# dfdazac/blp

Measured on AMD Instinct MI355X. Metric: scored triples/sec, all-entity eval (raw + filtered ranks, MRR + Hits@k), higher is better.
Workload: dtype f32; 1 GPU; fb15k237-transe; rel_model=transe, entities=14541, dim=128, triples_per_ranking_call=52870, filter_graph_edges=310116, parallelism=single GPU, ranks_in_process_group=1

## Files before the change

### blp_amd/csrc/rank_sad.hip

```cpp
#include <hip/hip_runtime.h>
#include <stddef.h>
#include <stdint.h>
#include <stdlib.h>

#include "exact_coop.h"
#include "knobs.h"
#include "launch.h"
#include "rank_common.h"
#include "sad_common.h"
#include "score_core.h"

#pragma clang fp contract(off)

namespace blp {


template <int D>
__global__ __launch_bounds__(256) void sad_range_kernel(const float* __restrict__ table, int64_t N, int64_t ld,
                                                        const QRows q_fixed,
                                                        const QRows q_rel, int64_t q_head, int64_t Q,
                                                        SadParams* __restrict__ partial) {
    SadRange range;
    const int64_t stride = (int64_t)gridDim.x * blockDim.x, t0 = (int64_t)blockIdx.x * blockDim.x + threadIdx.x;
    for (int64_t i = t0; i < N * (D / 4); i += stride) {
        const float4 v = *reinterpret_cast<const float4*>(table + (i / (D / 4)) * ld + (i % (D / 4)) * 4);
        range.see(v.x); range.see(v.y); range.see(v.z); range.see(v.w);
    }
    for (int64_t u = t0; u < Q * (D / 4); u += stride) {
        const bool head = u / (D / 4) < q_head;
        const float4 f = *reinterpret_cast<const float4*>(q_fixed.flat(4 * u, D));
        const float4 r = *reinterpret_cast<const float4*>(q_rel.flat(4 * u, D));
        range.see(sad_coef(f.x, r.x, head)); range.see(sad_coef(f.y, r.y, head));
        range.see(sad_coef(f.z, r.z, head)); range.see(sad_coef(f.w, r.w, head));
    }
    sad_range_block_store(range, partial);
}

constexpr int64_t kSFoldFinishBlocks = 1024;
constexpr int64_t kSFoldRangeBlocks = 256;

template <int D>
__device__ __forceinline__ void sad_quantize_table_tile(int64_t tile, const float* __restrict__ table, int64_t N,
                                                        int64_t ld, const SadParams* __restrict__ p,
                                                        uint4* __restrict__ cimg, unsigned* __restrict__ resid) {
    const SadScale sc = sad_scale(p);
    if (!sc.ok) return;
    const int row_in = threadIdx.x >> 2, part = threadIdx.x & 3;
    const int64_t row = tile * 64 + row_in;
    constexpr int F = D / 4;
    unsigned w[F / 2];
    float res = 0.f;
    bool outside = false;
    if (row < N) {
        const float* src = table + row * ld + part * F;
#pragma unroll
        for (int i = 0; i < F / 4; ++i) {
            const float4 v = *reinterpret_cast<const float4*>(src + 4 * i);
            w[2 * i] = sad_quant(v.x, sc, res, outside);
            w[2 * i] |= sad_quant(v.y, sc, res, outside) << 16;
            w[2 * i + 1] = sad_quant(v.z, sc, res, outside);
            w[2 * i + 1] |= sad_quant(v.w, sc, res, outside) << 16;
        }
    } else {
#pragma unroll
        for (int i = 0; i < F / 2; ++i) w[i] = 0;
    }
    res += __shfl_xor(res, 1);
    res += __shfl_xor(res, 2);
    outside |= (bool)__shfl_xor((int)outside, 1);
    outside |= (bool)__shfl_xor((int)outside, 2);
    if (part == 0)
        resid[row] = outside ? kSRowExact : (unsigned)(res * 1.0001f + kSResidSlack * D) + 1u;
    uint4* dst = cimg + (tile * (D / 8) + part * (F / 8)) * 64 + row_in;
#pragma unroll
    for (int i = 0; i < F / 8; ++i) dst[i * 64] = make_uint4(w[4 * i], w[4 * i + 1], w[4 * i + 2], w[4 * i + 3]);
}

template <int D>
__device__ __forceinline__ void sad_quantize_queries_block(int64_t vblock, int64_t vgrid, const QRows& q_fixed,
                                                           const QRows& q_rel, int64_t q_head,
                                                           int64_t Q, const float* __restrict__ key_true,
                                                           const SadParams* __restrict__ p,
                                                           unsigned* __restrict__ qimg,
                                                           int2* __restrict__ thr, unsigned* __restrict__ flags,
                                                           int64_t n_flag_words) {
    const int64_t i = vblock * 256 + threadIdx.x;
    for (int64_t j = i; j < n_flag_words; j += vgrid * 256) flags[j] = 0;
    const SadScale sc = sad_scale(p);
    if (!sc.ok) return;
    __shared__ float part_res[4], part_max[4];
    __shared__ int part_out[4];
    const bool live = i < Q * (D / 2);
    const int64_t q = live ? i / (D / 2) : Q - 1;
    const bool head = q < q_head;
    float res = 0.f, qmax = 0.f;
    bool outside = false;
    if (live) {
        const float2 f = *reinterpret_cast<const float2*>(q_fixed.flat(2 * i, D));
        const float2 r = *reinterpret_cast<const float2*>(q_rel.flat(2 * i, D));
        unsigned w = sad_quant(sad_coef(f.x, r.x, head), sc, res, outside);
        w |= sad_quant(sad_coef(f.y, r.y, head), sc, res, outside) << 16;
        qimg[i] = w;
        qmax = fmaxf(fmaxf(fabsf(f.x), fabsf(f.y)), fmaxf(fabsf(r.x), fabsf(r.y)));
    }
#pragma unroll
    for (int off = 1; off < (D / 2 < 64 ? D / 2 : 64); off <<= 1) {
        res += __shfl_xor(res, off);
        qmax = fmaxf(qmax, __shfl_xor(qmax, off));
        outside |= (bool)__shfl_xor((int)outside, off);
    }
    if constexpr (D / 2 > 64) {
        const int w = threadIdx.x >> 6;
        if ((threadIdx.x & 63) == 0) { part_res[w] = res; part_max[w] = qmax; part_out[w] = outside; }
        __syncthreads();
        res = part_res[w & ~1] + part_res[w | 1];
        qmax = fmaxf(part_max[w & ~1], part_max[w | 1]);
        outside = part_out[w & ~1] || part_out[w | 1];
    }
    if (live && i % (D / 2) == 0) {
        const double u = 5.9604644775390625e-8;
        const double dt = -(double)key_true[q], s = (double)sc.scale;
        const double M = (double)fmaxf(sad_range_maxabs(sc), qmax);
        const double band = (double)res * 1.0001 + 2.0 * kSResidSlack * D + 1.0;
        const double gamma = 1.05 * (D + 2) * u, rho = 6.0 * D * u * M;
        int t_lo = -1, t_hi = (int)kSThrMax;
        if (!outside && M < 3.0e38 && dt >= 0.0 && dt < 1.0e300) {
            const double lo_v = s * (dt - rho) / (1.0 + gamma) - band;
            const double hi_v = s * (dt + rho) / (1.0 - gamma) + band;
            if (lo_v > 2.0) t_lo = lo_v - 1.0 < (double)kSThrMax ? (int)(lo_v - 1.0) : (int)kSThrMax;
            if (hi_v + 2.0 < (double)kSThrMax) t_hi = (int)(hi_v + 2.0);
        }
        thr[q] = make_int2(t_lo, t_hi);
    }
}

template <int D>
__global__ __launch_bounds__(256) void sad_quantize_kernel(const float* __restrict__ table, int64_t N, int64_t ld,
                                                           SadParams* __restrict__ p, const SadParams* __restrict__ partial,
                                                           int n_partial, uint4* __restrict__ cimg,
                                                           unsigned* __restrict__ resid, unsigned table_blocks,
                                                           const QRows q_fixed, const QRows q_rel, int64_t q_head, int64_t Q,
                                                           const float* __restrict__ key_true, unsigned* __restrict__ qimg,
                                                           int2* __restrict__ thr, unsigned* __restrict__ flags,
                                                           int64_t n_flag_words) {
    __shared__ SadParams p_block;
    const SadParams* pp = p;
    if (n_partial > 0) {
        if (threadIdx.x < 64) {
            const SadParams r = sad_range_finish_wave(partial, n_partial, threadIdx.x);
            if (threadIdx.x == 0) {
                p_block = r;
                if (blockIdx.x == 0) *p = r;
            }
        }
        __syncthreads();
        pp = &p_block;
    }
    if (blockIdx.x < table_blocks)
        sad_quantize_table_tile<D>(blockIdx.x, table, N, ld, pp, cimg, resid);
    else
        sad_quantize_queries_block<D>(blockIdx.x - table_blocks, gridDim.x - table_blocks, q_fixed, q_rel, q_head, Q, key_true, pp,
                                      qimg, thr, flags, n_flag_words);
}

template <int D, int TPW>
struct SadTiles {
    unsigned v[TPW][D / 2];
    unsigned bias[TPW];
    unsigned long long exact_rows[TPW];
};

#ifndef BLP_SAD_CHUNK_BLOCK
#define BLP_SAD_CHUNK_BLOCK 4
#endif
constexpr unsigned kSadChunkBlock = BLP_SAD_CHUNK_BLOCK;

#ifndef BLP_SAD_INLINE_CAP
#define BLP_SAD_INLINE_CAP 256
#endif
constexpr unsigned kSInlineCap = BLP_SAD_INLINE_CAP;
static_assert(kSInlineCap <= kSQuota, "the pooled list is the four slices of pair_s");

#ifdef BLP_TIMING
__device__ unsigned long long g_sad_timing[4];
extern "C" int blp_debug_read_sad_timing(unsigned long long* out) {
    hipError_t err = hipMemcpyFromSymbol(out, HIP_SYMBOL(g_sad_timing), sizeof(g_sad_timing));
    unsigned long long zero[4] = {0, 0, 0, 0};
    if (err == hipSuccess) err = hipMemcpyToSymbol(HIP_SYMBOL(g_sad_timing), zero, sizeof(zero));
    return (int)err;
}
#endif

template <int D, int TPW>
__global__ __launch_bounds__(kSW * 64, (TPW * D / 2 <= 64 ? 5 : TPW * D / 2 <= 128 ? 3 : 2)) void rank_sad_kernel(
    const uint4* __restrict__ cimg, const unsigned* __restrict__ resid, int64_t n_rows, int n_groups, int q_per_group,
    const unsigned* __restrict__ qimg, const int2* __restrict__ thr, int64_t Q, int words_per_query,
    unsigned long long* __restrict__ acc,
    unsigned* __restrict__ flags, uint2* __restrict__ pairs, SadParams* __restrict__ params,
    const float* __restrict__ table, int64_t ld, const QRows q_fixed, const QRows q_rel, int64_t q_head,
    const float* __restrict__ key_true) {
    if (!sad_scale(params).ok) return;
#ifdef BLP_TIMING
    const unsigned long long clk0 = __builtin_readcyclecounter(), wall0 = __builtin_amdgcn_s_memrealtime();
#endif
    __shared__ int2 thr_s[kSChunk];
    __shared__ unsigned cnt[kSChunk];
    __shared__ uint2 pair_s[kSQuota];
    __shared__ unsigned wave_used[kSW], wave_base[kSW], ec_max_s;
    const int tid = threadIdx.x;
    const int wave = __builtin_amdgcn_readfirstlane(tid >> 6);
    const int lane = tid & 63;
    const unsigned n_blocks = gridDim.x, xcd = blockIdx.x & 7u, per_xcd = n_blocks >> 3, rem_b = n_blocks & 7u;
    const unsigned logical = (xcd < rem_b ? xcd * (per_xcd + 1) : rem_b * (per_xcd + 1) + (xcd - rem_b) * per_xcd) + (blockIdx.x >> 3);
    const unsigned n_chunks_all = n_blocks / (unsigned)n_groups;
    const unsigned per_cb = (unsigned)n_groups * kSadChunkBlock, cb = logical / per_cb, in_cb = logical % per_cb;
    const unsigned chunks_here = n_chunks_all - cb * kSadChunkBlock < kSadChunkBlock ? n_chunks_all - cb * kSadChunkBlock : kSadChunkBlock;
    const int group = (int)(in_cb / chunks_here);
    const int64_t q0 = (int64_t)(cb * kSadChunkBlock + in_cb % chunks_here) * q_per_group;
    const int nq = (int)(Q - q0 < q_per_group ? Q - q0 : q_per_group);

    for (int i = tid; i < kSChunk; i += kSW * 64) cnt[i] = 0;
    if (tid == 0) ec_max_s = 0;
    __syncthreads();

    SadTiles<D, TPW> c;
    const int64_t n_tiles = (n_rows + 63) / 64;
    const int64_t tile0 = ((int64_t)group * kSW + wave) * TPW;
    unsigned ec_max = 0;
    static_for<TPW>([&](auto tt) {
        constexpr int t = decltype(tt)::value;
        int64_t tile = tile0 + t;
        const bool exists = tile * 64 + lane < n_rows;
        tile = tile < n_tiles ? tile : n_tiles - 1;
        const unsigned ec = resid[tile * 64 + lane];
        const bool marked = exists && ec == kSRowExact;
        c.exact_rows[t] = __ballot(marked);
        c.bias[t] = exists ? (marked ? 0u : ec) : kSInvalid;
        ec_max = exists && !marked && ec > ec_max ? ec : ec_max;
        const uint4* src = cimg + tile * (D / 8) * 64 + lane;
        static_for<D / 8>([&](auto jj) {
            constexpr int j = decltype(jj)::value;
            const uint4 x = src[j * 64];
            c.v[t][4 * j] = x.x; c.v[t][4 * j + 1] = x.y; c.v[t][4 * j + 2] = x.z; c.v[t][4 * j + 3] = x.w;
        });
    });
#pragma unroll
    for (int off = 32; off > 0; off >>= 1) {
        const unsigned o = __shfl_xor(ec_max, off);
        ec_max = o > ec_max ? o : ec_max;
    }
    if (lane == 0) atomicMax(&ec_max_s, ec_max);
    __syncthreads();
    for (int i = tid; i < kSChunk; i += kSW * 64) {
        int2 t2 = i < nq ? thr[q0 + i] : make_int2(0, 0);
        const long long hi2 = (long long)t2.y + 2ll * ec_max_s;
        t2.y = hi2 < (long long)kSThrMax ? (int)hi2 : (int)kSThrMax;
        thr_s[i] = t2;
    }
    __syncthreads();

    unsigned my_pairs = 0;
    const float* row = reinterpret_cast<const float*>(qimg + q0 * (D / 2));
    sf16 cur = sload16<0>(row);
    sdrain(cur);
    for (int jb = 0; jb < nq; jb += 64) {
    const int jn = nq - jb < 64 ? nq - jb : 64;
    unsigned cnt_reg = 0;
    unsigned long long bit = 1;
    for (int j = jb; j < jb + jn; ++j, row += D / 2, bit <<= 1) {
        const float* next_row = row + D / 2;
        const int2 th = thr_s[j];
        unsigned sad[TPW];
        static_for<TPW>([&](auto tt) { sad[decltype(tt)::value] = c.bias[decltype(tt)::value]; });
        static_for<D / 32>([&](auto kk) {
            constexpr int k = decltype(kk)::value;
            sf16 nxt;
            if constexpr (k + 1 < D / 32) nxt = sload16<(k + 1) * 64>(row); else nxt = sload16<0>(next_row);
            if constexpr (k == 0) { if ((j & 3) == wave) stouch<D * 2>(row + 3 * (D / 2)); }
            static_for<16>([&](auto ii) {
                constexpr int i = decltype(ii)::value;
                const float qf = cur[i];
                const unsigned qv = __float_as_uint(qf);
                static_for<TPW>([&](auto tt) {
                    constexpr int t = decltype(tt)::value;
                    sad[t] = __builtin_amdgcn_sad_u16(qv, c.v[t][16 * k + i], sad[t]);
                });
            });
            sdrain(nxt);
            cur = nxt;
        });
        unsigned n_above = 0;
        static_for<TPW>([&](auto tt) {
            constexpr int t = decltype(tt)::value;
            const unsigned long long above = __ballot((int)sad[t] < th.x) & ~c.exact_rows[t];
            const unsigned long long und = (__ballot((int)sad[t] <= th.y) | c.exact_rows[t]) & ~above;
            unsigned n_t = __popcll(above);
            if (und) {
                const unsigned n = __popcll(und);
                if (my_pairs + n <= kSQuota / kSW) {
                    if ((und >> lane) & 1ull)
                        pair_s[wave * (kSQuota / kSW) + my_pairs + __popcll(und & ((1ull << lane) - 1ull))] =
                            make_uint2((unsigned)(q0 + j), (unsigned)((tile0 + t) * 64 + lane));
                    my_pairs += n;
                } else {
                    const int64_t tile = tile0 + t;
                    if (lane == 0) atomicOr(flags + (size_t)(q0 + j) * words_per_query + (tile >> 5), 1u << (tile & 31));
                    n_t = 0;
                }
            }
            n_above += n_t;
        });
        {
            unsigned long long saved;
            asm volatile("s_mov_b64 %1, exec\n\ts_mov_b64 exec, %3\n\tv_add_u32 %0, %0, %2\n\ts_mov_b64 exec, %1"
                         : "+v"(cnt_reg), "=&s"(saved) : "s"(n_above), "s"(bit));
        }
    }
    if (cnt_reg) atomicAdd(&cnt[jb + lane], cnt_reg);
    }
    __syncthreads();
    for (int i = tid; i < nq; i += kSW * 64) {
        const unsigned long long v = cnt[i];
        if (v) atomicAdd(acc + q0 + i, v | (v << 32));
    }
    if (lane == 0) wave_used[wave] = my_pairs;
    __syncthreads();
    unsigned start[kSW + 1];
    start[0] = 0;
#pragma unroll
    for (int w = 0; w < kSW; ++w) start[w + 1] = start[w] + __builtin_amdgcn_readfirstlane(wave_used[w]);
    const unsigned total = start[kSW];
    if (tid == 0 && total) atomicAdd(&params->n_listed, total);
    if (total <= kSInlineCap) {
        if (wave == 0) {
            for (unsigned base = 0; base < total; base += 64) {
                const bool live = base + lane < total;
                const unsigned t = live ? base + lane : base;
                const unsigned w = (unsigned)(t >= start[1]) + (unsigned)(t >= start[2]) + (unsigned)(t >= start[3]);
                const unsigned first = w == 0 ? start[0] : w == 1 ? start[1] : w == 2 ? start[2] : start[3];
                const uint2 p = pair_s[w * (kSQuota / kSW) + (t - first)];
                const int64_t q = p.x;
                const float key = transe_key_lane<D>(table + (int64_t)p.y * ld, q_fixed.row(q), q_rel.row(q), q < q_head);
                const float kt = key_true[q];
                const unsigned long long gt = live && key > kt, ge_ = live && key >= kt;
                if (gt | ge_) atomicAdd(acc + q, gt | (ge_ << 32));
            }
        }
    } else {
        if (tid == 0) {
            const unsigned base = atomicAdd(&params->n_pairs, total);
            for (int w = 0; w < kSW; ++w) wave_base[w] = base + start[w];
        }
        __syncthreads();
        for (int w = 0; w < kSW; ++w)
            for (unsigned i = tid; i < wave_used[w]; i += kSW * 64) pairs[wave_base[w] + i] = pair_s[w * (kSQuota / kSW) + i];
    }
#ifdef BLP_TIMING
    if (lane == 0) {
        atomicAdd(&g_sad_timing[0], __builtin_readcyclecounter() - clk0);
        atomicAdd(&g_sad_timing[1], __builtin_amdgcn_s_memrealtime() - wall0);
        atomicAdd(&g_sad_timing[2], 1ull);
    }
#endif
}

template <int D>
__global__ __launch_bounds__(64) void sad_refine_pairs_kernel(const float* __restrict__ table, int64_t ld,
                                                              const QRows q_fixed,
                                                              const QRows q_rel,
                                                              const float* __restrict__ key_true, int64_t q_head,
                                                              const uint2* __restrict__ pairs,
                                                              const SadParams* __restrict__ params,
                                                              unsigned long long* __restrict__ acc, const Gate gate) {
    if (gate_heavy(gate)) return;
    __shared__ __attribute__((aligned(16))) float slab[64 * kRefStride];
    const int lane = threadIdx.x;
    const int64_t n = params->n_pairs;
    for (int64_t base = (int64_t)blockIdx.x * 64; base < n; base += (int64_t)gridDim.x * 64) {
        const int64_t i = base + lane;
        const uint2 p = i < n ? pairs[i] : make_uint2(kSNoPair, 0u);
        const bool live = p.x != kSNoPair;
        const int64_t q = live ? p.x : 0;
        const bool head = q < q_head;
        const float key = transe_key_64<D>(table + (live ? (int64_t)p.y : 0) * ld, q_fixed.row(q), q_rel.row(q), head, slab, lane);
        const float kt = key_true[q];
        const unsigned long long gt = live && key > kt, ge_ = live && key >= kt;
        if (gt | ge_) atomicAdd(acc + q, gt | (ge_ << 32));
    }
}

template <int D>
__global__ __launch_bounds__(256) void sad_refine_tiles_kernel(const float* __restrict__ table, int64_t n_rows,
                                                               int64_t ld, const QRows q_fixed,
                                                               const QRows q_rel,
                                                               const float* __restrict__ key_true, int64_t q_head,
                                                               int64_t Q, int words_per_query,
                                                               const unsigned* __restrict__ flags,
                                                               const SadParams* __restrict__ params,
                                                               unsigned long long* __restrict__ acc, const Gate gate,
                                                               const FallbackPrep prep, int64_t q_tail) {
    if (gate_heavy(gate)) {
        fallback_prep<TRANSE, D>(prep, q_fixed, q_rel, q_head, q_tail);
        return;
    }
    __shared__ int list[kSweepQueries], n_list;
    const bool all = !sad_scale(params).ok;
    const int lane = threadIdx.x & 63;
    const int64_t q_base = (int64_t)blockIdx.x * kSweepQueries;
    const int n = flagged_queries(flags, q_base, Q, words_per_query, all, list, &n_list);
    for (int i = threadIdx.x >> 6; i < n; i += 4) {
    const int64_t q = q_base + list[i];
    const unsigned* row = flags + q * words_per_query;
    const float kt = key_true[q];
    const float* f = q_fixed.row(q);
    const float* rl = q_rel.row(q);
    unsigned gt = 0, ge = 0;
    for (int w0 = 0; w0 < words_per_query; w0 += 64) {
        const unsigned mine = w0 + lane < words_per_query ? (all ? 0xFFFFFFFFu : row[w0 + lane]) : 0u;
        unsigned long long nonzero = __ballot(mine != 0);
        while (nonzero) {
            const int src = __builtin_ctzll(nonzero);
            nonzero &= nonzero - 1;
            unsigned bits = __shfl(mine, src);
            const int64_t tile_base = (int64_t)(w0 + src) * 32;
            while (bits) {
                const int b = __builtin_ctz(bits);
                bits &= bits - 1;
                const int64_t r = (tile_base + b) * 64 + lane;
                const bool ok = r < n_rows;
                if (__ballot(ok) == 0) continue;
                float e[D];
                load_row<D>(e, table + (ok ? r : 0) * ld);
                const float key = q < q_head ? Scorer<TRANSE, HEAD, D>::template score<false>(e, LazyCoef<TRANSE, HEAD, D>{f, rl})
                                             : Scorer<TRANSE, TAIL, D>::template score<false>(e, LazyCoef<TRANSE, TAIL, D>{f, rl});
                gt += ok && key > kt;
                ge += ok && key >= kt;
            }
        }
    }
    if (__ballot(gt | ge) == 0) continue;
#pragma unroll
    for (int off = 32; off > 0; off >>= 1) {
        gt += __shfl_down(gt, off);
        ge += __shfl_down(ge, off);
    }
    if (lane == 0) atomicAdd(acc + q, (unsigned long long)gt | ((unsigned long long)ge << 32));
    }
}

static constexpr int sad_tiles_per_wave(int D) { return D <= 64 ? 2 : 1; }

struct SadWorkspace {
    float* key_true;
    unsigned long long* acc;
    SadParams* params; SadParams* partial; int2* thr; unsigned* qimg; uint4* cimg; unsigned* resid; unsigned* flags;
    uint2* pairs;
    float* fallback_coef;
    int64_t pass_groups;
    size_t bytes;
};

static int sad_queries_per_group(int D, int64_t N, int64_t Q) {
    const int64_t tiles_per_group = kSW * sad_tiles_per_wave(D);
    const int64_t n_groups = ((N + 63) / 64 + tiles_per_group - 1) / tiles_per_group;
    const int64_t resident = D >= 256 ? 256 * 3 : 256 * 5;
    const int64_t query_cycles = (int64_t)(D / 2) * sad_tiles_per_wave(D) * 17 / 4, setup_cycles = 12000;
    if (const int forced = (int)knob(KNOB_SAD_QUERIES_PER_GROUP))
        if (forced >= 16 && forced <= kSChunk && (forced & (forced - 1)) == 0) return forced;
    int best = kSChunk;
    int64_t best_cost = INT64_MAX;
    for (int per_group = kSChunk; per_group >= 16; per_group >>= 1) {
        const int64_t grid = n_groups * ((Q + per_group - 1) / per_group);
        const int64_t cost = ((grid + resident - 1) / resident) * (setup_cycles + per_group * query_cycles);
        if (cost < best_cost) { best_cost = cost; best = per_group; }
    }
    return best;
}

static int64_t sad_groups_per_pass(int D, int64_t N, int64_t Q) {
    const int64_t tiles_per_group = kSW * sad_tiles_per_wave(D);
    const int64_t n_groups = ((N + 63) / 64 + tiles_per_group - 1) / tiles_per_group;
    const int64_t per_group = sad_queries_per_group(D, N, Q);
    const int64_t n_chunks = (Q + per_group - 1) / per_group;
    const int64_t cap = (int64_t)256 << 20;
    int64_t by_pairs = cap / (kSQuota * 8) / (n_chunks > 0 ? n_chunks : 1);
    int64_t by_flags = cap / 4 / (Q > 0 ? Q : 1) * 32 / tiles_per_group;
    int64_t g = n_groups;
    if (g > by_pairs) g = by_pairs;
    if (g > by_flags) g = by_flags;
    if (const int64_t forced = knob(KNOB_SAD_PASS_GROUPS))
        if (forced > 0 && forced < g) g = forced;
    return g < 1 ? 1 : g;
}

static SadWorkspace carve_sad(void* base, int D, int64_t N, int64_t q_head, int64_t q_tail) {
    SadWorkspace w;
    const int64_t Q = q_head + q_tail;
    char* p = static_cast<char*>(base);
    size_t off = 0;
    w.key_true = reinterpret_cast<float*>(p + off);  off = align_up(off + (size_t)Q * 4, 256);
    w.acc = reinterpret_cast<unsigned long long*>(p + off);   off = align_up(off + (size_t)Q * 8, 256);
    w.params = reinterpret_cast<SadParams*>(p + off); off = align_up(off + sizeof(SadParams), 256);
    w.partial = reinterpret_cast<SadParams*>(p + off); off = align_up(off + sizeof(SadParams) * kSRangeBlocks, 256);
    w.thr = reinterpret_cast<int2*>(p + off);         off = align_up(off + (size_t)Q * 8, 256);
    w.qimg = reinterpret_cast<unsigned*>(p + off);    off = align_up(off + (size_t)(Q + 4) * (D / 2) * 4 + 64, 256);
    w.cimg = reinterpret_cast<uint4*>(p + off);       off = align_up(off + (size_t)((N + 63) / 64) * 64 * (D / 2) * 4, 256);
    w.resid = reinterpret_cast<unsigned*>(p + off);   off = align_up(off + (size_t)((N + 63) / 64) * 64 * 4, 256);
    w.pass_groups = sad_groups_per_pass(D, N, Q);
    const int64_t tiles_per_group = kSW * sad_tiles_per_wave(D);
    const int64_t words = (w.pass_groups * tiles_per_group + 31) / 32;
    w.flags = reinterpret_cast<unsigned*>(p + off); off = align_up(off + (size_t)Q * words * 4, 256);
    w.pairs = reinterpret_cast<uint2*>(p + off);
    const int64_t per_group = sad_queries_per_group(D, N, Q);
    off = align_up(off + (size_t)w.pass_groups * ((Q + per_group - 1) / per_group) * kSQuota * 8, 256);
    w.fallback_coef = nullptr;
    const int64_t n_groups_all = ((N + 63) / 64 + tiles_per_group - 1) / tiles_per_group;
    if (w.pass_groups >= n_groups_all && Q * N >= kFallbackMinPairs && Q <= 0x7fffffff / 2) {
        w.fallback_coef = reinterpret_cast<float*>(p + off);
        off = align_up(off + exact_fallback_coef_floats(D, q_head, q_tail) * 4, 256);
    }
    w.bytes = off;
    return w;
}

bool rank_sad_applicable(int model, int D, int64_t N, int64_t q_head, int64_t q_tail) {
    if (knob(KNOB_RANK_KERNEL) == 1) return false;
    const int64_t Q = q_head + q_tail;
    int64_t min_queries = kSadMinQueries;
    bool forced = false;
    if (const int64_t v = knob(KNOB_SAD_MIN_QUERIES)) { min_queries = v > 0 ? v : 1; forced = true; }
    if (model != TRANSE || !(D == 64 || D == 128 || D == 256) || Q < min_queries) return false;
    return forced || Q * N >= kSadMinPairs;
}

hipError_t sad_prepass_stats(int D, int64_t N, int64_t q_head, int64_t q_tail, const void* workspace, PrepassStats* out,
                             hipStream_t stream) {
    const SadWorkspace w = carve_sad(const_cast<void*>(workspace), D, N, q_head, q_tail);
    out->path = 1;
    const int64_t tiles_per_group = kSW * sad_tiles_per_wave(D);
    const int64_t words = (w.pass_groups * tiles_per_group + 31) / 32;
    unsigned long long host[3] = {0, 0, 0};
    const hipError_t err = launch_count_bits(w.flags, (q_head + q_tail) * words, w.pairs, &w.params->n_pairs, false, host, stream);
    out->flagged_rows = (long long)host[0] * 64;
    if (err != hipSuccess) return err;
    unsigned n_listed = 0;
    hipError_t err2 = hipMemcpyAsync(&n_listed, &w.params->n_listed, 4, hipMemcpyDeviceToHost, stream);
    if (err2 == hipSuccess) err2 = hipStreamSynchronize(stream);
    out->listed = (long long)n_listed;
    return err2;
}

size_t rank_sad_workspace_bytes(int model, int D, int64_t N, int64_t q_head, int64_t q_tail) {
    if (!rank_sad_applicable(model, D, N, q_head, q_tail)) return 0;
    return carve_sad(nullptr, D, N, q_head, q_tail).bytes;
}

template <int D>
static hipError_t rank_sad_impl(const float* table, int64_t N, int64_t ld, const QRows q_fixed, const QRows q_rel,
                                const QRows q_true, int64_t q_head, int64_t q_tail,
                                const FilterSpec& filter, int32_t* counts, void* workspace,
                                int n_cu, hipStream_t stream, hipEvent_t ev_start, hipEvent_t ev_stop) {
    constexpr int TPW = sad_tiles_per_wave(D);
    const int64_t Q = q_head + q_tail;
    SadWorkspace w = carve_sad(workspace, D, N, q_head, q_tail);
    hipError_t err = launch_true_keys(TRANSE, D, q_fixed, q_rel, q_head, q_tail, q_true, w.key_true, w.acc,
                                      stream);
    if (err != hipSuccess) return err;
    if (ev_start) (void)hipEventRecord(ev_start, stream);
    const int64_t n_tiles = (N + 63) / 64;
    const int64_t query_blocks = (Q * (D / 2) + 255) / 256;
    if (n_tiles + query_blocks > 0x7fffffff) return hipErrorInvalidValue;
    const bool fold_finish = n_tiles + query_blocks <= kSFoldFinishBlocks;
    int64_t range_blocks;
    {
        const int64_t items = N * (D / 4) > Q * D ? N * (D / 4) : Q * D, cap = fold_finish ? kSFoldRangeBlocks : kSRangeBlocks;
        range_blocks = (items + 255) / 256;
        range_blocks = range_blocks < cap ? (range_blocks > 0 ? range_blocks : 1) : cap;
        sad_range_kernel<D><<<dim3((unsigned)range_blocks), 256, 0, stream>>>(table, N, ld, q_fixed, q_rel, q_head, Q, w.partial);
        if (!fold_finish) sad_range_finish_kernel<<<1, 64, 0, stream>>>(w.partial, (int)range_blocks, w.params);
    }
    const int64_t first_rows = N < w.pass_groups * kSW * TPW * 64 ? N : w.pass_groups * kSW * TPW * 64;
    const int64_t first_groups = ((first_rows + 63) / 64 + kSW * TPW - 1) / (kSW * TPW);
    const int64_t first_words = (first_groups * kSW * TPW + 31) / 32;
    sad_quantize_kernel<D><<<dim3((unsigned)(n_tiles + query_blocks)), 256, 0, stream>>>(
        table, N, ld, w.params, w.partial, fold_finish ? (int)range_blocks : 0, w.cimg, w.resid, (unsigned)n_tiles, q_fixed, q_rel,
        q_head, Q, w.key_true, w.qimg, w.thr, w.flags, first_words * Q);

    const int64_t tiles_per_group = kSW * TPW;
    const int per_group = sad_queries_per_group(D, N, Q);
    const int64_t n_chunks = (Q + per_group - 1) / per_group;
    const int64_t pass_rows = w.pass_groups * tiles_per_group * 64;
    for (int64_t slab0 = 0; slab0 < N; slab0 += pass_rows) {
        const int64_t n_rows = N - slab0 < pass_rows ? N - slab0 : pass_rows;
        const int64_t slab_tiles = (n_rows + 63) / 64;
        const int64_t n_groups = (slab_tiles + tiles_per_group - 1) / tiles_per_group;
        const int words = (int)((n_groups * tiles_per_group + 31) / 32);
        const int64_t n_blocks = n_groups * n_chunks;
        if (slab0 > 0) {
            err = hipMemsetAsync(w.flags, 0, (size_t)Q * words * 4, stream);
            if (err != hipSuccess) return err;
            static_assert(offsetof(SadParams, n_listed) == offsetof(SadParams, n_pairs) + 4, "one memset clears both counters");
            err = hipMemsetAsync(&w.params->n_pairs, 0, 8, stream);
            if (err != hipSuccess) return err;
        }
        const float* slab = table + slab0 * ld;
        rank_sad_kernel<D, TPW><<<dim3((unsigned)n_blocks), kSW * 64, 0, stream>>>(
            w.cimg + (slab0 / 64) * (D / 8) * 64, w.resid + slab0, n_rows, (int)n_groups, per_group, w.qimg, w.thr, Q, words, w.acc,
            w.flags, w.pairs, w.params, slab, ld, q_fixed, q_rel, q_head, w.key_true);
        const int64_t pair_blocks = (n_blocks * kSQuota + 63) / 64;
        const Gate gate{w.fallback_coef ? &w.params->n_listed : nullptr, (unsigned)((n_blocks * kSQuota / 10 * 9) < 0xffffffffll ? n_blocks * kSQuota / 10 * 9 : 0xffffffffll)};
        sad_refine_pairs_kernel<D><<<dim3((unsigned)(pair_blocks < (int64_t)n_cu * 40 ? pair_blocks : (int64_t)n_cu * 40)), 64, 0, stream>>>(
            slab, ld, q_fixed, q_rel, w.key_true, q_head, w.pairs, w.params, w.acc, gate);
        sad_refine_tiles_kernel<D><<<dim3((unsigned)((Q + kSweepQueries - 1) / kSweepQueries)), 256, 0, stream>>>(
            slab, n_rows, ld, q_fixed, q_rel, w.key_true, q_head, Q, words, w.flags, w.params, w.acc, gate,
            FallbackPrep{w.fallback_coef, w.acc}, q_tail);
        if (gate.counter) {
            err = launch_exact_fallback(TRANSE, D, table, N, ld, q_fixed, q_rel, q_head, q_tail, w.fallback_coef, w.key_true, w.acc, gate,
                                        n_cu, stream);
            if (err != hipSuccess) return err;
        }
    }
    if (ev_stop) (void)hipEventRecord(ev_stop, stream);
    err = launch_filter_finalize(TRANSE, D, table, N, ld, q_fixed, q_rel, w.key_true, q_head, q_tail, filter,
                                 w.acc, counts, stream);
    return err != hipSuccess ? err : hipGetLastError();
}

hipError_t launch_rank_all_sad(int D, const float* table, int64_t N, int64_t ld, const QRows q_fixed,
                               const QRows q_rel, const QRows q_true, int64_t q_head,
                               int64_t q_tail, const FilterSpec& filter, int32_t* counts,
                               void* workspace, int n_cu, hipStream_t stream, hipEvent_t ev_start,
                               hipEvent_t ev_stop) {
#define BLP_SAD_CASE(DD)                                                                                          \
    if (D == DD)                                                                                                  \
        return rank_sad_impl<DD>(table, N, ld, q_fixed, q_rel, q_true, q_head, q_tail, filter,          \
                                 counts, workspace, n_cu, stream, ev_start, ev_stop);
    BLP_SAD_CASE(64) BLP_SAD_CASE(128) BLP_SAD_CASE(256)
#undef BLP_SAD_CASE
    return hipErrorInvalidValue;
}

}
```

Baseline: 506.2 billion scored triples/s.

## Vectorize query quantization and load per-query thresholds via scalar loads

```diff
diff --git a/blp_amd/csrc/rank_sad.hip b/blp_amd/csrc/rank_sad.hip
--- a/blp_amd/csrc/rank_sad.hip
+++ b/blp_amd/csrc/rank_sad.hip
@@ -88,36 +88,40 @@
     for (int64_t j = i; j < n_flag_words; j += vgrid * 256) flags[j] = 0;
     const SadScale sc = sad_scale(p);
     if (!sc.ok) return;
-    __shared__ float part_res[4], part_max[4];
-    __shared__ int part_out[4];
-    const bool live = i < Q * (D / 2);
-    const int64_t q = live ? i / (D / 2) : Q - 1;
+    const bool live = i < Q * (D / 8);
+    const int64_t q = live ? i / (D / 8) : Q - 1;
     const bool head = q < q_head;
     float res = 0.f, qmax = 0.f;
     bool outside = false;
     if (live) {
-        const float2 f = *reinterpret_cast<const float2*>(q_fixed.flat(2 * i, D));
-        const float2 r = *reinterpret_cast<const float2*>(q_rel.flat(2 * i, D));
-        unsigned w = sad_quant(sad_coef(f.x, r.x, head), sc, res, outside);
-        w |= sad_quant(sad_coef(f.y, r.y, head), sc, res, outside) << 16;
-        qimg[i] = w;
-        qmax = fmaxf(fmaxf(fabsf(f.x), fabsf(f.y)), fmaxf(fabsf(r.x), fabsf(r.y)));
+        const float* fp = q_fixed.flat(8 * i, D);
+        const float* rp = q_rel.flat(8 * i, D);
+        const float4 f0 = *reinterpret_cast<const float4*>(fp), f1 = *reinterpret_cast<const float4*>(fp + 4);
+        const float4 r0 = *reinterpret_cast<const float4*>(rp), r1 = *reinterpret_cast<const float4*>(rp + 4);
+        float p0 = 0.f, p1 = 0.f, p2 = 0.f, p3 = 0.f;
+        uint4 w;
+        w.x = sad_quant(sad_coef(f0.x, r0.x, head), sc, p0, outside);
+        w.x |= sad_quant(sad_coef(f0.y, r0.y, head), sc, p0, outside) << 16;
+        w.y = sad_quant(sad_coef(f0.z, r0.z, head), sc, p1, outside);
+        w.y |= sad_quant(sad_coef(f0.w, r0.w, head), sc, p1, outside) << 16;
+        w.z = sad_quant(sad_coef(f1.x, r1.x, head), sc, p2, outside);
+        w.z |= sad_quant(sad_coef(f1.y, r1.y, head), sc, p2, outside) << 16;
+        w.w = sad_quant(sad_coef(f1.z, r1.z, head), sc, p3, outside);
+        w.w |= sad_quant(sad_coef(f1.w, r1.w, head), sc, p3, outside) << 16;
+        reinterpret_cast<uint4*>(qimg)[i] = w;
+        res = (p0 + p1) + (p2 + p3);
+        qmax = fmaxf(fmaxf(fmaxf(fabsf(f0.x), fabsf(f0.y)), fmaxf(fabsf(f0.z), fabsf(f0.w))),
+                     fmaxf(fmaxf(fabsf(f1.x), fabsf(f1.y)), fmaxf(fabsf(f1.z), fabsf(f1.w))));
+        qmax = fmaxf(qmax, fmaxf(fmaxf(fmaxf(fabsf(r0.x), fabsf(r0.y)), fmaxf(fabsf(r0.z), fabsf(r0.w))),
+                                 fmaxf(fmaxf(fabsf(r1.x), fabsf(r1.y)), fmaxf(fabsf(r1.z), fabsf(r1.w)))));
     }
 #pragma unroll
-    for (int off = 1; off < (D / 2 < 64 ? D / 2 : 64); off <<= 1) {
+    for (int off = 1; off < D / 8; off <<= 1) {
         res += __shfl_xor(res, off);
         qmax = fmaxf(qmax, __shfl_xor(qmax, off));
         outside |= (bool)__shfl_xor((int)outside, off);
     }
-    if constexpr (D / 2 > 64) {
-        const int w = threadIdx.x >> 6;
-        if ((threadIdx.x & 63) == 0) { part_res[w] = res; part_max[w] = qmax; part_out[w] = outside; }
-        __syncthreads();
-        res = part_res[w & ~1] + part_res[w | 1];
-        qmax = fmaxf(part_max[w & ~1], part_max[w | 1]);
-        outside = part_out[w & ~1] || part_out[w | 1];
-    }
-    if (live && i % (D / 2) == 0) {
+    if (live && i % (D / 8) == 0) {
         const double u = 5.9604644775390625e-8;
         const double dt = -(double)key_true[q], s = (double)sc.scale;
         const double M = (double)fmaxf(sad_range_maxabs(sc), qmax);
@@ -191,6 +195,15 @@
 }
 #endif
 
+typedef int si2 __attribute__((ext_vector_type(2)));
+
+__device__ __forceinline__ si2 sload2(const int2* base, unsigned byte_off) {
+    si2 v;
+    asm volatile("s_load_dwordx2 %0, %1, %2" : "=s"(v) : "s"(base), "s"(byte_off) : "memory");
+    return v;
+}
+__device__ __forceinline__ void sdrain(sf16& a, si2& b) { asm volatile("s_waitcnt lgkmcnt(0)" : "+s"(a), "+s"(b) : : "memory"); }
+
 template <int D, int TPW>
 __global__ __launch_bounds__(kSW * 64, (TPW * D / 2 <= 64 ? 5 : TPW * D / 2 <= 128 ? 3 : 2)) void rank_sad_kernel(
     const uint4* __restrict__ cimg, const unsigned* __restrict__ resid, int64_t n_rows, int n_groups, int q_per_group,
@@ -203,7 +216,6 @@
 #ifdef BLP_TIMING
     const unsigned long long clk0 = __builtin_readcyclecounter(), wall0 = __builtin_amdgcn_s_memrealtime();
 #endif
-    __shared__ int2 thr_s[kSChunk];
     __shared__ unsigned cnt[kSChunk];
     __shared__ uint2 pair_s[kSQuota];
     __shared__ unsigned wave_used[kSW], wave_base[kSW], ec_max_s;
@@ -251,16 +263,11 @@
     }
     if (lane == 0) atomicMax(&ec_max_s, ec_max);
     __syncthreads();
-    for (int i = tid; i < kSChunk; i += kSW * 64) {
-        int2 t2 = i < nq ? thr[q0 + i] : make_int2(0, 0);
-        const long long hi2 = (long long)t2.y + 2ll * ec_max_s;
-        t2.y = hi2 < (long long)kSThrMax ? (int)hi2 : (int)kSThrMax;
-        thr_s[i] = t2;
-    }
-    __syncthreads();
+    const int ec_max2 = __builtin_amdgcn_readfirstlane((int)(2u * ec_max_s));
 
     unsigned my_pairs = 0;
     const float* row = reinterpret_cast<const float*>(qimg + q0 * (D / 2));
+    const int2* thr_q = thr + q0;
     sf16 cur = sload16<0>(row);
     sdrain(cur);
     for (int jb = 0; jb < nq; jb += 64) {
@@ -269,13 +276,14 @@
     unsigned long long bit = 1;
     for (int j = jb; j < jb + jn; ++j, row += D / 2, bit <<= 1) {
         const float* next_row = row + D / 2;
-        const int2 th = thr_s[j];
+        si2 th;
         unsigned sad[TPW];
         static_for<TPW>([&](auto tt) { sad[decltype(tt)::value] = c.bias[decltype(tt)::value]; });
         static_for<D / 32>([&](auto kk) {
             constexpr int k = decltype(kk)::value;
             sf16 nxt;
             if constexpr (k + 1 < D / 32) nxt = sload16<(k + 1) * 64>(row); else nxt = sload16<0>(next_row);
+            if constexpr (k + 1 == D / 32) th = sload2(thr_q, (unsigned)j * 8u);
             if constexpr (k == 0) { if ((j & 3) == wave) stouch<D * 2>(row + 3 * (D / 2)); }
             static_for<16>([&](auto ii) {
                 constexpr int i = decltype(ii)::value;
@@ -286,14 +294,15 @@
                     sad[t] = __builtin_amdgcn_sad_u16(qv, c.v[t][16 * k + i], sad[t]);
                 });
             });
-            sdrain(nxt);
+            if constexpr (k + 1 < D / 32) sdrain(nxt); else sdrain(nxt, th);
             cur = nxt;
         });
+        const int t_lo = th.x, t_hi = th.y + ec_max2 < (int)kSThrMax ? th.y + ec_max2 : (int)kSThrMax;
         unsigned n_above = 0;
         static_for<TPW>([&](auto tt) {
             constexpr int t = decltype(tt)::value;
-            const unsigned long long above = __ballot((int)sad[t] < th.x) & ~c.exact_rows[t];
-            const unsigned long long und = (__ballot((int)sad[t] <= th.y) | c.exact_rows[t]) & ~above;
+            const unsigned long long above = __ballot((int)sad[t] < t_lo) & ~c.exact_rows[t];
+            const unsigned long long und = (__ballot((int)sad[t] <= t_hi) | c.exact_rows[t]) & ~above;
             unsigned n_t = __popcll(above);
             if (und) {
                 const unsigned n = __popcll(und);
@@ -568,9 +577,9 @@
     if (err != hipSuccess) return err;
     if (ev_start) (void)hipEventRecord(ev_start, stream);
     const int64_t n_tiles = (N + 63) / 64;
-    const int64_t query_blocks = (Q * (D / 2) + 255) / 256;
+    const int64_t query_blocks = (Q * (D / 8) + 255) / 256;
     if (n_tiles + query_blocks > 0x7fffffff) return hipErrorInvalidValue;
-    const bool fold_finish = n_tiles + query_blocks <= kSFoldFinishBlocks;
+    const bool fold_finish = n_tiles + (Q * (D / 2) + 255) / 256 <= kSFoldFinishBlocks;
     int64_t range_blocks;
     {
         const int64_t items = N * (D / 4) > Q * D ? N * (D / 4) : Q * D, cap = fold_finish ? kSFoldRangeBlocks : kSRangeBlocks;
```

Result: no change. 510.9 billion scored triples/s, median of 6 (+0.9%).
